# Daaohame/RAHT-3DGS-codec

Measured on AMD Instinct MI355X. Metric: M-Gaussians/s fwd+inv RAHT, 59-ch SH3 3DGS, higher is better.
Workload: dtype f32 (xyz columns: f64); 1 GPU; cfg3: 2999072 Gaussians (3000000 draws/GPU, J=12, 59 channels), fwd RAHT + quantize/reorder + dequantize/un-reorder + inv RAHT (quantization fused into the transform kernels); the 3 xyz columns carried in float64 inside the same launches (raht_fwd_quant_mixed / raht_dequant_inv_mixed): the reference's integers on every column; rows_per_gpu=2999072, channels=59, depth_J=12, engine=tile, quantize=True, parallelism=1 GPU, world=1

## Files before the change

raht-3dgs-codec_amd/csrc/transform_mx.hip:

```cpp
#include "raht_common.h"
#include "raht_device.h"
#include "tile_engine.h"
#include "tile_host.h"

#include <algorithm>
#include <cstdlib>
#include <string>
#include <type_traits>
#include <vector>

namespace raht {

#ifdef RAHT_PHASE_CLOCKS
constexpr int MX_CLK_TILES = 4096, MX_CLK_SLOTS = 12;
__device__ unsigned long long g_phase_clk_mx[MX_CLK_TILES][MX_CLK_SLOTS];
#define MX_STAMP(k) do { if (IDENT && threadIdx.x == 0 && tile_id < MX_CLK_TILES) g_phase_clk_mx[tile_id][k] = __builtin_readcyclecounter(); } while (0)
#else
#define MX_STAMP(k) do { } while (0)
#endif

constexpr int MX_MAX_WIDE = 4;
constexpr int MX_THREADS = 512;
constexpr int MX_TOP_THREADS = 1024;
constexpr int MX_TOP_SLOTS = RAHT_TOP_MAX_ROWS / MX_TOP_THREADS;

struct StepTableMX {
    StepTable f;
    double w[MX_MAX_WIDE];
};

static size_t tile_lds_bytes_mx(int R, int NF, int nwide)
{
    const size_t data = (size_t)R * NF * 16 + (((size_t)R * nwide * 8 + 15) & ~(size_t)15);
    const size_t meta = (size_t)R * (16 + 4 + 4);
    const size_t surv = ((size_t)R * 2 + 15) & ~(size_t)15;
    return data + meta + surv;
}

struct MxPtrs {
    const double *in_w;
    double *out_w;
    double *wsn_w;
    double *root_w;
    const uint32_t *prog;
    uint32_t prog_stride, prog_ab;
    int prog_compact;
};

struct MxMultiQ {
    int k;
    uint32_t fast_div;
    double step[MULTI_Q_MAX];
    int32_t *Q[MULTI_Q_MAX];
};

template <bool INV, bool IDENT, int SLOTS, bool ROOTS, bool MULTI = false, bool SQ = false>
__device__ __forceinline__ void tile_body_mx(const TileArgs<float> &A, const MxPtrs &P, const StepTableMX &ST, const int64_t tile_id,
                                             const MxMultiQ *MQ = nullptr)
{
    extern __shared__ __align__(16) unsigned char smem[];
    typedef RegChunk<float> V16;
    typedef RegChunk<double> W16;
    typedef RegChunk<int32_t> I16;
    const int R = A.R;
    const int tid0 = threadIdx.x;
    const int nthreads = blockDim.x, nwv = nthreads >> 6;
    const int nwide = A.nwide;
    const int lgw = nwide > 2 ? 2 : nwide - 1;
    const int Df = A.D;
    const int Fp = A.Dp, NF = Fp >> 2;
    const int lg = A.lg, lr = 6 - A.lg;
    const uint32_t NFm = ((1u << 20) + (uint32_t)NF - 1) / (uint32_t)NF;
    auto sync_lds = [&]() { asm volatile("s_waitcnt lgkmcnt(0)\n\ts_barrier" ::: "memory"); };
    auto wait_landed = [&]() { asm volatile("s_waitcnt vmcnt(0)" ::: "memory"); };

    size_t off = 0;
    float *ftile = (float *)smem; off += (size_t)R * Fp * 4;
    double *wd = (double *)(smem + off); off += ((size_t)R * nwide * 8 + 15) & ~(size_t)15;
    W16 *rec_ab = (W16 *)(smem + off); off += (size_t)R * 16;
    uint32_t *rec_pj = (uint32_t *)(smem + off); off += (size_t)R * 4;
    int32_t *sdst = (int32_t *)(smem + off); off += (size_t)R * 4;
    uint16_t *ssurv = (uint16_t *)(smem + off);

    auto lane_geom = [&](int tid, int &lane, int &wid, int &g, int &c4, int &fl, int &sp, int &goff, bool &head) {
        lane = tid & 63;
        wid = __builtin_amdgcn_readfirstlane(tid >> 6);
        g = lane >> lg;
        c4 = lane & ((1 << lg) - 1);
        fl = min(c4, NF - 1);
        head = c4 == 0;
        sp = fl;
        goff = min(fl * 4, Df - 4);
    };
    float my_step[4], my_rcp[4], tab_step[4];
    auto fetch_steps = [&](int place) {
        const int g0 = ST.f.n == 1 ? 0 : min(place * 4, Df - 4);
#pragma unroll
        for (int i = 0; i < 4; ++i) tab_step[i] = ST.f.v[g0 + i];
    };
    auto use_steps = [&]() {
#pragma unroll
        for (int i = 0; i < 4; ++i) {
            my_step[i] = ST.f.n == 1 ? ST.f.v[0] : tab_step[i];
            my_rcp[i] = refined_rcp(my_step[i]);
        }
    };

    int tid = tid0;
    asm volatile("" : "+v"(tid));
    int lane, wid, g, c4, fl, sp, goff; bool head;
    lane_geom(tid, lane, wid, g, c4, fl, sp, goff, head);
    const int64_t e0 = tile_id * R;
    const int nt = (int)min((int64_t)R, A.n_entries - e0);
    MX_STAMP(0);
    if constexpr (!MULTI) fetch_steps(fl);

    const uint32_t *pg = P.prog + (uint64_t)tile_id * P.prog_stride;
    const int end_v = ((const uint16_t *)pg)[lane];
    const int endm_v = lane ? ((const uint16_t *)pg)[lane - 1] : 0;
    uint32_t surv_raw = A.surv_off ? A.surv_off[tile_id + (tid0 & 1)] : 0u;
    uint32_t m_rw[SLOTS], m_rec[SLOTS];
    W16 m_ab[SLOTS];
#pragma unroll
    for (int s = 0; s < SLOTS; ++s) {
        const int j = tid0 + s * nthreads;
        m_rw[s] = 0; m_rec[s] = 0; m_ab[s].v[0] = 0.0; m_ab[s].v[1] = 0.0;
        if (j < nt) {
            m_rw[s] = pg[32 + j];
            m_rec[s] = pg[32 + R + j];
            if (!P.prog_compact) m_ab[s] = ((const W16 *)(pg + P.prog_ab))[j];
        }
    }
    auto early_loads_landed = [&]() {
        asm volatile("" : "+v"(surv_raw));
        if constexpr (!MULTI) asm volatile("" : "+v"(tab_step[0]), "+v"(tab_step[1]), "+v"(tab_step[2]), "+v"(tab_step[3]));
    };
    auto fin_of = [&](uint32_t rw) { return (rw >> 31) != 0 || (A.last_stage && !ROOTS); };
    auto write_dst = [&]() {
#pragma unroll
        for (int s = 0; s < SLOTS; ++s) {
            const int j = tid0 + s * nthreads;
            if (j < nt) sdst[j] = (int32_t)((m_rw[s] & 0x7fffffffu) | (fin_of(m_rw[s]) ? 0x80000000u : 0u));
        }
    };
    auto write_survivors = [&](uint32_t n_merged) {
#pragma unroll
        for (int s = 0; s < SLOTS; ++s) {
            const uint32_t k = (uint32_t)(tid0 + s * nthreads);
            if (k >= n_merged && k < (uint32_t)nt) ssurv[k - n_merged] = (uint16_t)m_rec[s];
        }
    };
    auto write_records = [&](uint32_t n_merged) {
#pragma unroll
        for (int s = 0; s < SLOTS; ++s) {
            const uint32_t k = (uint32_t)(tid0 + s * nthreads);
            if (k < n_merged) {
                uint32_t pj = m_rec[s];
                W16 ab = m_ab[s];
                if (P.prog_compact) {
                    const uint32_t j = pj & 1023u, l = (pj >> 10) & 1023u, r = (pj >> 20) & 1023u;
                    const double w0 = (double)(int)l, w1 = (double)(int)r;
                    const double den = w0 + w1;
                    ab.v[0] = sqrt(w0 / den);
                    ab.v[1] = sqrt(w1 / den);
                    pj = (j - l) | (j << 16);
                }
                rec_ab[k] = ab;
                rec_pj[k] = pj;
            }
        }
    };

    auto load_linear = [&](const float *dst, int chunks, const float *src) {
        const uint32_t lds0 = (uint32_t)(uintptr_t)(__attribute__((address_space(3))) const void *)dst;
        for (int it = wid; (it << 6) < chunks; it += nwv) {
            const int c = (it << 6) + lane;
            if (c < chunks) glds16<0>(src + (uint32_t)c * 4u, lds0 + ((uint32_t)it << 10));
        }
    };
    auto load_caller_rows = [&](int rows, auto src) {
        const uint32_t lds0 = (uint32_t)(uintptr_t)(__attribute__((address_space(3))) const void *)ftile;
        const int total = rows * NF;
        for (int it = wid; (it << 6) < total; it += nwv) {
            const int c = (it << 6) + lane;
            const int jr = (int)(((uint32_t)c * NFm) >> 20), ch = c - jr * NF;
            if (c < total) { const void *a = src(jr, (uint32_t)min(ch * 4, Df - 4)); if (a) glds16<1>(a, lds0 + ((uint32_t)it << 10)); }
        }
    };
    auto widen_row = [&](int j) {
        double *row = wd + __mul24(j, nwide);
        const V16 raw = *(const V16 *)(ftile + __mul24(j, Fp));
        double d[4];
#pragma unroll
        for (int i = 0; i < 4; ++i) d[i] = i < nwide ? (double)raw.v[i] : 0.0;
#pragma unroll
        for (int i = 0; i < 4; ++i) if (i < nwide) row[i] = d[i];
    };

    if constexpr (!INV) {
        if constexpr (IDENT) {
            const uint32_t ldc = (uint32_t)A.ld_in;
            const float *src = A.in + e0 * (int64_t)ldc;
            load_caller_rows(nt, [&](int jr, uint32_t go) { return row_at(src, (uint32_t)jr, ldc, go); });
        } else {
            load_linear(ftile, nt * NF, A.in + e0 * (int64_t)Fp);
            load_linear((const float *)wd, (nt * nwide + 1) >> 1, (const float *)(P.in_w + e0 * (int64_t)nwide));
        }
        MX_STAMP(9);
        const uint32_t n_merged = (uint32_t)__builtin_amdgcn_readlane(end_v, 63);
        write_dst();
        write_survivors(n_merged);
        write_records(n_merged);
        MX_STAMP(1);
        wait_landed();
        early_loads_landed();
        sync_lds();
        MX_STAMP(2);
        if constexpr (IDENT) {
#pragma unroll
            for (int s = 0; s < SLOTS; ++s) {
                const int j = tid + s * nthreads;
                if (j < nt) widen_row(j);
            }
            sync_lds();
        }
        MX_STAMP(3);
        MX_STAMP(4);
    } else {
        const uint32_t n_merged = (uint32_t)__builtin_amdgcn_readlane(end_v, 63);
        write_dst();
        write_survivors(n_merged);
        MX_STAMP(1);
        sync_lds();
        MX_STAMP(2);
        load_caller_rows(nt, [&](int jr, uint32_t go) -> const void * {
            const uint32_t d = (uint32_t)sdst[jr];
            return (d >> 31) ? (const void *)row_far((const int32_t *)A.Q, d & 0x7fffffffu, (uint32_t)A.ldq, go) : nullptr; });
        write_records(n_merged);
        const uint32_t surv_base = (uint32_t)__builtin_amdgcn_readlane((int)surv_raw, 0);
        const uint32_t surv_cnt = (uint32_t)__builtin_amdgcn_readlane((int)surv_raw, 1) - surv_base;
        if (!A.last_stage) {
            if (c4 < NF) for (uint32_t it = wid; (it << lr) < surv_cnt; it += nwv) {
                const uint32_t qc = min((it << lr) + g, surv_cnt - 1);
                const V16 x = ld_chunk<float>(row_at((const float *)A.wsn + (int64_t)surv_base * Fp, qc, (uint32_t)Fp, (uint32_t)(fl * 4)));
                *(V16 *)&ftile[__mul24((int)ssurv[qc], Fp) + fl * 4] = x;
            }
            for (uint32_t c = (uint32_t)tid; c < surv_cnt * (uint32_t)nwide; c += (uint32_t)nthreads) {
                const uint32_t qc = c / (uint32_t)nwide, i = c - qc * (uint32_t)nwide;
                wd[__mul24((int)ssurv[qc], nwide) + i] = P.wsn_w[(int64_t)surv_base * nwide + c];
            }
        } else if (ROOTS) {
            if (c4 < NF) for (uint32_t it = wid; (it << lr) < surv_cnt; it += nwv) {
                const uint32_t qc = min((it << lr) + g, surv_cnt - 1);
                const V16 x = ld_chunk<float>(A.root_buf + (int64_t)(surv_base + qc) * Df + goff);
                *(V16 *)&ftile[__mul24((int)ssurv[qc], Fp) + fl * 4] = x;
            }
            for (uint32_t c = (uint32_t)tid; c < surv_cnt * (uint32_t)nwide; c += (uint32_t)nthreads) {
                const uint32_t qc = c / (uint32_t)nwide, i = c - qc * (uint32_t)nwide;
                wd[__mul24((int)ssurv[qc], nwide) + i] = P.root_w[(int64_t)surv_base * nwide + c];
            }
        }
        MX_STAMP(3);
        wait_landed();
        early_loads_landed();
        sync_lds();
        MX_STAMP(4);
        use_steps();
#pragma unroll
        for (int s = 0; s < SLOTS; ++s) {
            const int j = tid0 + s * nthreads;
            if (j < nt && fin_of(m_rw[s])) {
                double *row = wd + __mul24(j, nwide);
                const I16 raw = *(const I16 *)(ftile + __mul24(j, Fp));
#pragma unroll
                for (int i = 0; i < 4; ++i) if (i < nwide) row[i] = (double)raw.v[i] * ST.w[i];
            }
        }
        if (A.last_stage && !ROOTS) {
            const uint32_t n_fin = (uint32_t)nt - n_merged;
            if (c4 < NF) for (uint32_t it = wid; (it << lr) < n_fin; it += nwv) {
                const uint32_t qc = (it << lr) + g;
                if (qc < n_fin) {
                    V16 *pr = (V16 *)&ftile[__mul24((int)ssurv[qc], Fp) + fl * 4];
                    const I16 raw = *(const I16 *)pr;
                    V16 x;
#pragma unroll
                    for (int i = 0; i < 4; ++i)
                        x.v[i] = (head && i < nwide) ? __int_as_float(raw.v[i]) : (float)raw.v[i] * my_step[i];
                    *pr = x;
                }
            }
        }
        sync_lds();
    }
    MX_STAMP(5);
    {
        const uint32_t stride = (uint32_t)(nwv << lr);
        const uint32_t gw = (uint32_t)lane >> lgw, cw = (uint32_t)min(lane & ((1 << lgw) - 1), nwide - 1);
        const uint32_t bw = 64u >> lgw;
        const uint32_t cf = (uint32_t)fl * 4u;
        bool chained = false;
        const int loff_v = endm_v, hist_v = end_v - endm_v;
        uint64_t mask = __ballot(hist_v > 0);
        while (mask) {
            const int l = INV ? (63 - __clzll((long long)mask)) : (__ffsll((long long)mask) - 1);
            mask &= ~(1ull << l);
            const uint32_t base = (uint32_t)__builtin_amdgcn_readlane(loff_v, l), cnt = (uint32_t)__builtin_amdgcn_readlane(hist_v, l);
            auto apply_f = [&](auto UC, uint32_t mb) {
                constexpr int U = decltype(UC)::value;
                W16 ab[U];
                uint32_t pj[U];
#pragma unroll
                for (int u = 0; u < U; ++u) { const uint32_t m = base + min(mb + u * stride + g, cnt - 1); pj[u] = rec_pj[m]; ab[u] = rec_ab[m]; }
                uint32_t ip[U], ij[U];
                V16 x0[U], x1[U];
#pragma unroll
                for (int u = 0; u < U; ++u) { ip[u] = __umul24(pj[u] & 0xffffu, (uint32_t)Fp) + cf; ij[u] = __umul24(pj[u] >> 16, (uint32_t)Fp) + cf; }
#pragma unroll
                for (int u = 0; u < U; ++u) { x0[u] = *(const V16 *)&ftile[ip[u]]; x1[u] = *(const V16 *)&ftile[ij[u]]; }
                if constexpr (INV) {
#pragma unroll
                    for (int u = 0; u < U; ++u) {
#pragma unroll
                        for (int i = 0; i < 4; ++i) x1[u].v[i] = (float)__float_as_int(x1[u].v[i]) * my_step[i];
                    }
                }
#pragma unroll
                for (int u = 0; u < U; ++u) {
                    const float ca = (float)ab[u].v[0], cb = (float)ab[u].v[1];
                    V16 lo, hi;
#pragma unroll
                    for (int i = 0; i < 4; ++i) {
                        if (!INV) {
                            lo.v[i] = ca * x0[u].v[i] + cb * x1[u].v[i];
                            hi.v[i] = ca * x1[u].v[i] - cb * x0[u].v[i];
                        } else {
                            lo.v[i] = ca * x0[u].v[i] - cb * x1[u].v[i];
                            hi.v[i] = cb * x0[u].v[i] + ca * x1[u].v[i];
                        }
                    }
                    if (u == 0 || mb + u * stride < cnt) { *(V16 *)&ftile[ip[u]] = lo; *(V16 *)&ftile[ij[u]] = hi; }
                }
            };
            auto pass_f = [&](auto UC) {
                constexpr int U = decltype(UC)::value;
                for (uint32_t mb = (uint32_t)(wid << lr); mb < cnt; mb += stride * U) apply_f(UC, mb);
            };
            auto apply_w = [&](uint32_t m0) {
                const uint32_t m = base + min(m0 + gw, cnt - 1);
                const uint32_t pj = rec_pj[m];
                const W16 ab = rec_ab[m];
                const uint32_t ip = __umul24(pj & 0xffffu, (uint32_t)nwide) + cw, ij = __umul24(pj >> 16, (uint32_t)nwide) + cw;
                const double d0 = wd[ip], d1 = wd[ij];
                const double ca = ab.v[0], cb = ab.v[1];
                double lo, hi;
                if (!INV) {
                    lo = ca * d0 + cb * d1;
                    hi = ca * d1 - cb * d0;
                } else {
                    lo = ca * d0 - cb * d1;
                    hi = cb * d0 + ca * d1;
                }
                wd[ip] = lo; wd[ij] = hi;
            };
            if (cnt <= (1u << lr)) {
                if (wid == 0) pass_f(std::integral_constant<int, 1>());
                else if (wid == 1) { for (uint32_t m0 = 0; m0 < cnt; m0 += bw) apply_w(m0); }
                chained = true;
            } else {
                if (chained) { __syncthreads(); chained = false; }
                if (cnt <= stride) pass_f(std::integral_constant<int, 1>());
                else pass_f(std::integral_constant<int, TILE_ROUND_U>());
                for (uint32_t m0 = (uint32_t)(nwv - 1 - wid) * bw; m0 < cnt; m0 += (uint32_t)nwv * bw) apply_w(m0);
                __syncthreads();
            }
        }
        if (chained) __syncthreads();
    }

    MX_STAMP(6);
    {
        int tid5 = tid0;
        asm volatile("" : "+v"(tid5));
        lane_geom(tid5, lane, wid, g, c4, fl, sp, goff, head);
    }
    const bool rowlane = c4 < NF;
    if constexpr (INV) {
        if constexpr (IDENT) {
            float *base = A.out + e0 * A.ld_out;
            double acc[4] = {0.0, 0.0, 0.0, 0.0};
            const float *rbase = SQ ? A.ref + e0 * A.ld_ref : nullptr;
            if (rowlane) for (int it = wid; (it << lr) < nt; it += 2 * nwv) {
                int j[2]; V16 x[2]; double w[2][4] = {};
                V16 c[2];
                if constexpr (SQ) {
#pragma unroll
                    for (int u = 0; u < 2; ++u)
                        c[u] = ld_chunk<float, true>(row_at(rbase, (uint32_t)min(((it + u * nwv) << lr) + g, nt - 1), (uint32_t)A.ld_ref, (uint32_t)goff));
                }
#pragma unroll
                for (int u = 0; u < 2; ++u) {
                    j[u] = min(((it + u * nwv) << lr) + g, nt - 1);
                    x[u] = *(const V16 *)&ftile[__mul24(j[u], Fp) + sp * 4];
                }
                if (head) {
#pragma unroll
                    for (int u = 0; u < 2; ++u) {
#pragma unroll
                        for (int i = 0; i < 4; ++i) w[u][i] = wd[__mul24(j[u], nwide) + min(i, nwide - 1)];
                    }
                }
                asm volatile("" : "+v"(w[0][0]), "+v"(w[0][1]), "+v"(w[0][2]), "+v"(w[0][3]), "+v"(w[1][0]), "+v"(w[1][1]), "+v"(w[1][2]), "+v"(w[1][3]));
#pragma unroll
                for (int u = 0; u < 2; ++u) {
#pragma unroll
                    for (int i = 0; i < 4; ++i) { const float f = (float)w[u][i]; x[u].v[i] = (head && i < nwide) ? f : x[u].v[i]; }
                    asm volatile("" : "+v"(x[u].v[0]), "+v"(x[u].v[1]), "+v"(x[u].v[2]), "+v"(x[u].v[3]));
                    if constexpr (SQ) {
                        if (u == 0 || ((it + nwv) << lr) < nt) {
                            if (A.out) st_chunk<float, true>(row_at(base, (uint32_t)j[u], (uint32_t)A.ld_out, (uint32_t)goff), x[u]);
                            if (((it + u * nwv) << lr) + g < nt) {
#pragma unroll
                                for (int i = 0; i < 4; ++i) { const float d = x[u].v[i] - c[u].v[i]; acc[i] += (double)d * (double)d; }
                            }
                        }
                    } else if (u == 0 || ((it + nwv) << lr) < nt) {
                        st_chunk<float, true>(row_at(base, (uint32_t)j[u], (uint32_t)A.ld_out, (uint32_t)goff), x[u]);
                    }
                }
            }
            if constexpr (SQ) {
#pragma unroll
                for (int i = 0; i < 4; ++i) {
                    for (int sh = 1 << lg; sh < 64; sh <<= 1) acc[i] += __shfl_xor(acc[i], sh, 64);
                }
                __syncthreads();
                double *sacc = (double *)smem;
                if (g == 0 && rowlane) {
#pragma unroll
                    for (int i = 0; i < 4; ++i) sacc[(wid * NF + c4) * 4 + i] = acc[i];
                }
                __syncthreads();
                if (tid0 < NF * 4) {
                    double t = 0.0;
                    for (int w = 0; w < nwv; ++w) t += sacc[w * NF * 4 + tid0];
                    A.sq_part[tile_id * (NF * 4) + tid0] = t;
                }
            }
        } else {
            float *bf = A.out + e0 * (int64_t)Fp;
            double *bw_ = P.out_w + e0 * (int64_t)nwide;
            for (int c = tid; c < nt * NF; c += nthreads) st_chunk<float>(bf + c * 4, *(const V16 *)&ftile[c * 4]);
            for (int c = tid; c < nt * nwide; c += nthreads) bw_[c] = wd[c];
        }
    } else {
        if (!A.last_stage || ROOTS) {
            const uint32_t surv_base = (uint32_t)__builtin_amdgcn_readlane((int)surv_raw, 0);
            const uint32_t surv_cnt = (uint32_t)__builtin_amdgcn_readlane((int)surv_raw, 1) - surv_base;
            constexpr bool to_roots = ROOTS;
            float *bf = to_roots ? A.root_buf + (int64_t)surv_base * Df : A.wsn + (int64_t)surv_base * Fp;
            double *bw_ = (to_roots ? P.root_w : P.wsn_w) + (int64_t)surv_base * nwide;
            const uint32_t ldb = (uint32_t)(to_roots ? Df : Fp), cb = (uint32_t)(to_roots ? goff : fl * 4);
            if (c4 < NF) for (uint32_t it = wid; (it << lr) < surv_cnt; it += nwv) {
                const uint32_t q = min((it << lr) + g, surv_cnt - 1);
                const V16 x = *(const V16 *)&ftile[__mul24((int)ssurv[q], Fp) + fl * 4];
                st_chunk<float>(row_at(bf, q, ldb, cb), x);
            }
            for (uint32_t c = (uint32_t)tid; c < surv_cnt * (uint32_t)nwide; c += (uint32_t)nthreads) {
                const uint32_t q = c / (uint32_t)nwide, i = c - q * (uint32_t)nwide;
                bw_[c] = wd[__mul24((int)ssurv[q], nwide) + i];
            }
        }
        if constexpr (MULTI) {
            int32_t *qa = (int32_t *)rec_ab;
            auto store_step = [&](auto fast_div, int32_t *Qd) {
                if (rowlane) for (int it = wid; (it << lr) < nt; it += 2 * nwv) {
                    int jc[2]; V16 x[2]; I16 qi[2] = {}; uint32_t dv[2];
#pragma unroll
                    for (int u = 0; u < 2; ++u) {
                        jc[u] = min(((it + u * nwv) << lr) + g, nt - 1);
                        x[u] = *(const V16 *)&ftile[__mul24(jc[u], Fp) + sp * 4];
                        dv[u] = (uint32_t)sdst[jc[u]];
                    }
                    if (head) {
#pragma unroll
                        for (int u = 0; u < 2; ++u) {
#pragma unroll
                            for (int i = 0; i < 4; ++i) qi[u].v[i] = qa[__mul24(jc[u], nwide) + min(i, nwide - 1)];
                        }
                    }
                    asm volatile("" : "+v"(x[0].v[0]), "+v"(x[1].v[0]), "+v"(qi[0].v[0]), "+v"(qi[0].v[1]), "+v"(qi[0].v[2]), "+v"(qi[0].v[3]),
                                 "+v"(qi[1].v[0]), "+v"(qi[1].v[1]), "+v"(qi[1].v[2]), "+v"(qi[1].v[3]));
#pragma unroll
                    for (int u = 0; u < 2; ++u) {
                        I16 qv;
#pragma unroll
                        for (int i = 0; i < 4; ++i) {
                            const int32_t q = quantize_one(x[u].v[i], my_step[i], my_rcp[i], decltype(fast_div)::value);
                            qv.v[i] = (head && i < nwide) ? qi[u].v[i] : q;
                        }
                        asm volatile("" : "+v"(qv.v[0]), "+v"(qv.v[1]), "+v"(qv.v[2]), "+v"(qv.v[3]));
                        if ((dv[u] >> 31) && (u == 0 || ((it + nwv) << lr) < nt))
                            st_chunk<int32_t, true>(row_far(Qd, dv[u] & 0x7fffffffu, (uint32_t)A.ldq, (uint32_t)goff), qv);
                    }
                }
            };
            for (int kk = 0; kk < MQ->k; ++kk) {
                const double sw = MQ->step[kk];
#pragma unroll
                for (int s = 0; s < SLOTS; ++s) {
                    const int j = tid0 + s * nthreads;
                    if (j < nt && ((uint32_t)sdst[j] >> 31)) {
                        const double *row = &wd[__mul24(j, nwide)];
                        int32_t *qrow = &qa[__mul24(j, nwide)];
#pragma unroll
                        for (int i = 0; i < 4; ++i) if (i < nwide) qrow[i] = quantize_one_f64(row[i], sw);
                    }
                }
                sync_lds();
                const float sf = (float)sw, rf = refined_rcp(sf);
#pragma unroll
                for (int i = 0; i < 4; ++i) { my_step[i] = sf; my_rcp[i] = rf; }
                if ((MQ->fast_div >> kk) & 1u) store_step(std::true_type(), MQ->Q[kk]);
                else store_step(std::false_type(), MQ->Q[kk]);
                sync_lds();
            }
        } else {
            MX_STAMP(10);
#pragma unroll
            for (int s = 0; s < SLOTS; ++s) {
                const int j = tid0 + s * nthreads;
                if (j < nt && ((uint32_t)sdst[j] >> 31)) {
                    double *row = &wd[__mul24(j, nwide)];
                    double d[4] = {0.0, 0.0, 0.0, 0.0};
#pragma unroll
                    for (int i = 0; i < 4; ++i) if (i < nwide) d[i] = row[i];
                    asm volatile("" ::: "memory");
                    int32_t *qrow = (int32_t *)row;
#pragma unroll
                    for (int i = 0; i < 4; ++i) if (i < nwide) qrow[i] = quantize_one_f64(d[i], ST.w[i]);
                }
            }
            sync_lds();
            MX_STAMP(7);
            use_steps();
#ifdef RAHT_PHASE_CLOCKS
            asm volatile("" :: "v"(my_step[0]), "v"(my_rcp[3]));
#endif
            MX_STAMP(11);
            auto store_final = [&](auto fast_div) {
                if (rowlane) for (int it = wid; (it << lr) < nt; it += 2 * nwv) {
                    int jc[2]; V16 x[2]; I16 qi[2] = {}; uint32_t dv[2];
#pragma unroll
                    for (int u = 0; u < 2; ++u) {
                        jc[u] = min(((it + u * nwv) << lr) + g, nt - 1);
                        x[u] = *(const V16 *)&ftile[__mul24(jc[u], Fp) + sp * 4];
                        dv[u] = (uint32_t)sdst[jc[u]];
                    }
                    if (head) {
#pragma unroll
                        for (int u = 0; u < 2; ++u) {
                            const int32_t *qrow = (const int32_t *)&wd[__mul24(jc[u], nwide)];
#pragma unroll
                            for (int i = 0; i < 4; ++i) qi[u].v[i] = qrow[min(i, nwide - 1)];
                        }
                    }
                    asm volatile("" : "+v"(x[0].v[0]), "+v"(x[1].v[0]), "+v"(qi[0].v[0]), "+v"(qi[0].v[1]), "+v"(qi[0].v[2]), "+v"(qi[0].v[3]),
                                 "+v"(qi[1].v[0]), "+v"(qi[1].v[1]), "+v"(qi[1].v[2]), "+v"(qi[1].v[3]));
#pragma unroll
                    for (int u = 0; u < 2; ++u) {
                        I16 qv;
#pragma unroll
                        for (int i = 0; i < 4; ++i) {
                            const int32_t q = quantize_one(x[u].v[i], my_step[i], my_rcp[i], decltype(fast_div)::value);
                            qv.v[i] = (head && i < nwide) ? qi[u].v[i] : q;
                        }
                        asm volatile("" : "+v"(qv.v[0]), "+v"(qv.v[1]), "+v"(qv.v[2]), "+v"(qv.v[3]));
                        if ((dv[u] >> 31) && (u == 0 || ((it + nwv) << lr) < nt))
                            st_chunk<int32_t, true>(row_far(A.Q, dv[u] & 0x7fffffffu, (uint32_t)A.ldq, (uint32_t)goff), qv);
                    }
                }
            };
            if (ST.f.fast_div) store_final(std::true_type()); else store_final(std::false_type());
        }
    }
    MX_STAMP(8);
}

template <bool INV, bool IDENT, int SLOTS>
__global__ __launch_bounds__(MX_THREADS, 6) void tile_kernel_mx(const TileArgs<float> A, const MxPtrs P, const StepTableMX ST)
{
    tile_body_mx<INV, IDENT, SLOTS, false>(A, P, ST, (int64_t)blockIdx.x);
}
template <bool INV, bool IDENT, int SLOTS>
__global__ __launch_bounds__(MX_THREADS, 6) void tile_kernel_mx_roots(const TileArgs<float> A, const MxPtrs P, const StepTableMX ST)
{
    tile_body_mx<INV, IDENT, SLOTS, true>(A, P, ST, (int64_t)blockIdx.x);
}
template <bool IDENT, int SLOTS>
__global__ __launch_bounds__(MX_THREADS, 6) void tile_kernel_mx_multi(const TileArgs<float> A, const MxPtrs P, const StepTableMX ST, const MxMultiQ M)
{
    tile_body_mx<false, IDENT, SLOTS, false, true, false>(A, P, ST, (int64_t)blockIdx.x, &M);
}
template <int SLOTS>
__global__ __launch_bounds__(MX_THREADS, 6) void tile_kernel_mx_sq(const TileArgs<float> A, const MxPtrs P, const StepTableMX ST)
{
    tile_body_mx<true, true, SLOTS, false, false, true>(A, P, ST, (int64_t)blockIdx.x);
}

struct TileBatchMX {
    TileArgs<float> a[BATCH_MAX];
    MxPtrs p[BATCH_MAX];
    uint32_t first_tile[BATCH_MAX + 1];
    int n;
};
static_assert(sizeof(TileBatchMX) + sizeof(StepTableMX) <= 4096, "tile_kernel_mx_batch: arguments exceed the 4 KB kernarg segment");

template <bool INV, bool IDENT, int SLOTS>
__global__ __launch_bounds__(MX_THREADS, 6) void tile_kernel_mx_batch(const TileBatchMX B, const StepTableMX ST)
{
    int s = 0;
#pragma unroll
    for (int q = 1; q < BATCH_MAX; ++q) s += (q < B.n && blockIdx.x >= B.first_tile[q]) ? 1 : 0;
    tile_body_mx<INV, IDENT, SLOTS, false>(B.a[s], B.p[s], ST, (int64_t)(blockIdx.x - B.first_tile[s]));
}

struct TopArgsMX {
    const float *in_rows;  int64_t ld_in;
    const float *in_img; const double *in_img_w;
    float *out_rows;       int64_t ld_out;
    float *out_img; double *out_img_w;
    int32_t *Q;            int64_t ldq;
    const uint32_t *e_pos;
    const uint32_t *pj;
    const float *ab32;  const double *ab64;
    int n, n_merges, D, nwide, Fp;
    const uint32_t *lev;
    int nlev, nbig;
    uint32_t small_start;
    const uint32_t *root_rank;
    float *root_f; double *root_w;
};

template <bool WIDE, bool INV, bool ROOTS, bool MULTI = false>
__device__ __forceinline__ void top_body_mx(const TopArgsMX &A, const StepTableMX &ST, const int chunk, const MxMultiQ *MQ = nullptr)
{
    typedef typename std::conditional<WIDE, double, float>::type T;
    constexpr int VN = WIDE ? 2 : 4;
    typedef RegChunk<T> V16;
    extern __shared__ __align__(16) unsigned char smem[];
    V16 *tile = (V16 *)smem;
    __shared__ uint32_t s_lev[2 * 64];
    const int tid = threadIdx.x;
    const int nwide = A.nwide;
    const int goff = WIDE ? 2 * chunk : min(chunk * 4, A.D - 4);
    const int ioff = chunk * 4;
    const int n = A.n, nm = A.n_merges;
    if (tid < 2 * A.nlev) s_lev[tid] = A.lev[tid];
    const T *ab = WIDE ? (const T *)A.ab64 : (const T *)A.ab32;
    const int n_small = nm - (int)A.small_start;
    uint32_t *s_pj = (uint32_t *)(smem + (size_t)n * 16);
    T *s_ab = (T *)(s_pj + ((n_small + 3) & ~3));
    for (int i = tid; i < n_small; i += MX_TOP_THREADS) {
        s_pj[i] = A.pj[A.small_start + i];
        s_ab[2 * i] = ab[2 * (A.small_start + i)];
        s_ab[2 * i + 1] = ab[2 * (A.small_start + i) + 1];
    }
    T my_step[VN];
    float my_rcp[VN];
    bool live[VN];
#pragma unroll
    for (int i = 0; i < VN; ++i) {
        if constexpr (WIDE) { live[i] = goff + i < nwide; my_step[i] = live[i] ? ST.w[goff + i] : 1.0; my_rcp[i] = 1.0f; }
        else { live[i] = !(chunk == 0 && i < nwide); my_step[i] = ST.f.v[ST.f.n == 1 ? 0 : goff + i]; my_rcp[i] = refined_rcp(my_step[i]); }
    }
    uint32_t pj[MX_TOP_SLOTS];
    T ra[MX_TOP_SLOTS], rb[MX_TOP_SLOTS];
#pragma unroll
    for (int k = 0; k < MX_TOP_SLOTS; ++k) {
        const int idx = min(k * MX_TOP_THREADS + tid, max(nm - 1, 0));
        pj[k] = A.pj[idx]; ra[k] = ab[2 * idx]; rb[k] = ab[2 * idx + 1];
    }
    uint32_t m_dst[MX_TOP_SLOTS], m_rr[MX_TOP_SLOTS];
#pragma unroll
    for (int k = 0; k < MX_TOP_SLOTS; ++k) {
        m_dst[k] = A.e_pos[min(k * MX_TOP_THREADS + tid, n - 1)];
        m_rr[k] = ROOTS ? A.root_rank[min(k * MX_TOP_THREADS + tid, n - 1)] : 0xffffffffu;
    }
#pragma unroll
    for (int k = 0; k < MX_TOP_SLOTS; ++k) {
        const int e = k * MX_TOP_THREADS + tid;
        if (e >= n) continue;
        V16 v;
        if constexpr (!INV) {
            if (A.in_img) {
                if constexpr (WIDE) {
#pragma unroll
                    for (int i = 0; i < VN; ++i) v.v[i] = live[i] ? A.in_img_w[(int64_t)e * nwide + goff + i] : 0.0;
                } else {
                    v = *(const V16 *)(A.in_img + (int64_t)e * A.Fp + ioff);
                }
            } else if constexpr (WIDE) {
#pragma unroll
                for (int i = 0; i < VN; ++i) v.v[i] = live[i] ? (double)A.in_rows[(int64_t)e * A.ld_in + goff + i] : 0.0;
            } else {
                v = ld_chunk<float>(A.in_rows + (int64_t)e * A.ld_in + goff);
            }
        } else if (m_rr[k] != 0xffffffffu) {
            if constexpr (WIDE) {
#pragma unroll
                for (int i = 0; i < VN; ++i) v.v[i] = live[i] ? A.root_w[(int64_t)m_rr[k] * nwide + goff + i] : 0.0;
            } else {
                v = ld_chunk<float>(A.root_f + (int64_t)m_rr[k] * A.D + goff);
            }
        } else {
            const int32_t *q = A.Q + (int64_t)m_dst[k] * A.ldq + goff;
            if constexpr (WIDE) {
#pragma unroll
                for (int i = 0; i < VN; ++i) v.v[i] = live[i] ? (double)q[i] * my_step[i] : 0.0;
            } else {
                const RegChunk<int32_t> raw = ld_chunk<int32_t>(q);
#pragma unroll
                for (int i = 0; i < VN; ++i) v.v[i] = (float)raw.v[i] * my_step[i];
            }
        }
        tile[e] = v;
    }
    __syncthreads();

    auto butterfly = [&](uint32_t rec, T a, T b) {
        const uint32_t ip = rec & 0xffffu, ij = rec >> 16;
        const V16 x0 = tile[ip], x1 = tile[ij];
        V16 vlo, vhi;
#pragma unroll
        for (int i = 0; i < VN; ++i) {
            if (!INV) {
// ... 608 lines not shown
}

template <bool INV>
static int run_batch_mx(const char *what, int n, raht_plan *const *plans, const MxIO *ios, int D, const double *steps, int n_steps,
                        int n_wide, hipStream_t s)
{
    std::vector<MxScene> scn((size_t)n);
    for (int i = 0; i < n; ++i) {
        const MxIO &io = ios[i];
        const void *a = INV ? (const void *)io.Q : (const void *)io.C_in, *b = INV ? (const void *)io.C_out : (const void *)io.Q;
        RAHT_RET(mx_batch_check_plan(what, i, plans[i], a, b, D, INV ? io.ldq : io.ldc, INV ? io.ldc : io.ldq, steps, n_steps, n_wide));
    }
    std::vector<size_t> first((size_t)n + 1, 0);
    for (int i = 0; i < n; ++i) {
        MxScene &S = scn[(size_t)i];
        S.p = plans[i]; S.io = ios[i];
        Schedule *sc = nullptr;
        RAHT_RET(mx_setup(S.p, D, n_wide, std::max(S.io.ldc, S.io.ldq), s, &sc, S.g));
        S.sc = mx_batchable(S.p, sc) ? sc : nullptr;
        first[(size_t)i + 1] = first[(size_t)i] + (S.sc ? S.sc->stages.size() : 0);
    }
    std::vector<MxStageLaunch> prep(first[(size_t)n]);
    for (int i = 0; i < n; ++i) {
        const MxScene &S = scn[(size_t)i];
        if (!S.sc) continue;
        for (int k = 0; k < (int)S.sc->stages.size(); ++k) {
            const int rc = prepare_stage_mx<INV>(S.p, *S.sc, k, S.io, D, S.g, prep[first[(size_t)i] + (size_t)k]);
            if (rc != RAHT_OK) {
                const std::string msg = raht_last_error();
                set_error("%s: %s (scene %d)", what, msg.c_str(), i);
                return rc;
            }
        }
    }
    StepTableMX stp;
    fill_steps_mx(stp, steps, n_steps, n_wide);
    auto stage_of = [&](int i, int k) -> const MxStageLaunch & { return prep[first[(size_t)i] + (size_t)k]; };
    auto single = [&](int i) -> int {
        const MxIO &io = scn[(size_t)i].io;
        if constexpr (INV) return dequant_inv_mixed_impl(scn[(size_t)i].p, io.Q, io.ldq, D, steps, n_steps, n_wide, io.C_out, io.ldc, (raht_stream_t)s);
        else return fwd_quant_mixed_impl(scn[(size_t)i].p, io.C_in, io.ldc, D, steps, n_steps, n_wide, io.Q, io.ldq, (raht_stream_t)s);
    };
    auto tile = [&](int m, const int *idx, int k) -> int {
        if (m == 1) return launch_prepared_mx<INV>(scn[(size_t)idx[0]].p, k, scn[(size_t)idx[0]].io, stage_of(idx[0], k), scn[(size_t)idx[0]].g, stp, s);
        const MxStageLaunch *Ls[BATCH_MAX];
        for (int q = 0; q < m; ++q) Ls[q] = &stage_of(idx[q], k);
        return launch_tile_batch_mx<INV>(m, Ls, k == 0, stp, s);
    };
    auto top = [&](int m, const int *idx, int k) -> int {
        if (m == 1) return launch_prepared_mx<INV>(scn[(size_t)idx[0]].p, k, scn[(size_t)idx[0]].io, stage_of(idx[0], k), scn[(size_t)idx[0]].g, stp, s);
        const MxStageLaunch *Ls[BATCH_MAX];
        for (int q = 0; q < m; ++q) Ls[q] = &stage_of(idx[q], k);
        return launch_top_batch_mx<INV>(m, Ls, scn[(size_t)idx[0]].g.NCp, stp, s);
    };
    BatchCounts cnt;
    return group_mx_scenes<INV>(n, scn.data(), cnt, single, tile, top);
}

static int mixed_batch_stats_impl(int n, raht_plan *const *plans, int D, int n_wide, int inverse, int *tile_launches, int *top_launches,
                                  int *single_scene_calls)
{
    const char *what = "raht_mixed_batch_stats";
    if (n < 1 || !plans || !tile_launches || !top_launches || !single_scene_calls || D < 1 || n_wide < 1 || n_wide > MX_MAX_WIDE || n_wide > D) {
        set_error("%s: bad argument", what);
        return RAHT_ERR_INVALID;
    }
    RAHT_RET(check_batch_plans(what, n, plans));
    std::vector<MxScene> scn((size_t)n);
    for (int i = 0; i < n; ++i) {
        MxScene &S = scn[(size_t)i];
        S.p = plans[i];
        RAHT_RET(check_plan_device(S.p, what));
        if (S.p->row_map) { set_error("%s: not available for row-mapped plans (scene %d)", what, i); return RAHT_ERR_UNSUPPORTED; }
        Schedule *sc = nullptr;
        RAHT_RET(mx_setup(S.p, D, n_wide, D, nullptr, &sc, S.g));
        S.sc = mx_batchable(S.p, sc) ? sc : nullptr;
    }
    BatchCounts cnt;
    auto none1 = [](int) { return (int)RAHT_OK; };
    auto none3 = [](int, const int *, int) { return (int)RAHT_OK; };
    if (inverse) RAHT_RET((group_mx_scenes<true>(n, scn.data(), cnt, none1, none3, none3)));
    else RAHT_RET((group_mx_scenes<false>(n, scn.data(), cnt, none1, none3, none3)));
    *tile_launches = cnt.tile; *top_launches = cnt.top; *single_scene_calls = cnt.single;
    return RAHT_OK;
}

}

using namespace raht;

extern "C" {

int raht_fwd_quant_mixed(const raht_plan *plan, const float *C, int64_t ldc, int D, const double *steps, int n_steps, int n_wide,
                         int32_t *Q, int64_t ldq, raht_stream_t stream)
{
    return guarded("raht_fwd_quant_mixed", [&]() { return fwd_quant_mixed_impl(plan, C, ldc, D, steps, n_steps, n_wide, Q, ldq, stream); });
}

int raht_dequant_inv_mixed(const raht_plan *plan, const int32_t *Q, int64_t ldq, int D, const double *steps, int n_steps, int n_wide,
                           float *C, int64_t ldc, raht_stream_t stream)
{
    return guarded("raht_dequant_inv_mixed", [&]() { return dequant_inv_mixed_impl(plan, Q, ldq, D, steps, n_steps, n_wide, C, ldc, stream); });
}

int raht_fwd_quant_mixed_multi(const raht_plan *plan, const float *C, int64_t ldc, int D, const double *steps, int k, int n_wide,
                               int32_t *const *Q, int64_t ldq, raht_stream_t stream)
{
    return guarded("raht_fwd_quant_mixed_multi", [&]() { return fwd_quant_mixed_multi_impl(plan, C, ldc, D, steps, k, n_wide, Q, ldq, stream); });
}

int raht_dequant_inv_mixed_sqdiff(const raht_plan *plan, const int32_t *Q, int64_t ldq, int D, const double *steps, int n_steps,
                                  int n_wide, const float *C_ref, int64_t ld_ref, float *C_rec, int64_t ldc, double *sqdiff,
                                  raht_stream_t stream)
{
    return guarded("raht_dequant_inv_mixed_sqdiff", [&]() {
        return dequant_inv_mixed_sqdiff_impl(plan, Q, ldq, D, steps, n_steps, n_wide, C_ref, ld_ref, C_rec, ldc, sqdiff, stream); });
}

int raht_fwd_quant_mixed_batch(int n, raht_plan *const *plans, const float *const *C, const int64_t *ldc, int D,
                               const double *steps, int n_steps, int n_wide, int32_t *const *Q, const int64_t *ldq, raht_stream_t stream)
{
    const char *what = "raht_fwd_quant_mixed_batch";
    return guarded(what, [&]() -> int {
        RAHT_RET(mx_batch_check_args(what, n, plans, (const void *const *)C, ldc, (const void *const *)Q, ldq, D, steps, n_steps, n_wide));
        std::vector<MxIO> ios((size_t)n);
        for (int i = 0; i < n; ++i) { MxIO &io = ios[(size_t)i]; io.C_in = C[i]; io.ldc = ldc[i]; io.Q = Q[i]; io.ldq = ldq[i]; }
        return run_batch_mx<false>(what, n, plans, ios.data(), D, steps, n_steps, n_wide, (hipStream_t)stream);
    });
}

int raht_dequant_inv_mixed_batch(int n, raht_plan *const *plans, const int32_t *const *Q, const int64_t *ldq, int D,
                                 const double *steps, int n_steps, int n_wide, float *const *C, const int64_t *ldc, raht_stream_t stream)
{
    const char *what = "raht_dequant_inv_mixed_batch";
    return guarded(what, [&]() -> int {
        RAHT_RET(mx_batch_check_args(what, n, plans, (const void *const *)Q, ldq, (const void *const *)C, ldc, D, steps, n_steps, n_wide));
        std::vector<MxIO> ios((size_t)n);
        for (int i = 0; i < n; ++i) { MxIO &io = ios[(size_t)i]; io.C_out = C[i]; io.ldc = ldc[i]; io.Q = const_cast<int32_t *>(Q[i]); io.ldq = ldq[i]; }
        return run_batch_mx<true>(what, n, plans, ios.data(), D, steps, n_steps, n_wide, (hipStream_t)stream);
    });
}

int raht_mixed_batch_stats(int n, raht_plan *const *plans, int D, int n_wide, int inverse, int *tile_launches, int *top_launches,
                           int *single_scene_calls)
{
    return guarded("raht_mixed_batch_stats", [&]() {
        return mixed_batch_stats_impl(n, plans, D, n_wide, inverse, tile_launches, top_launches, single_scene_calls); });
}

#ifdef RAHT_PHASE_CLOCKS
int raht_debug_read_phase_clocks_mx(unsigned long long *dst, int n_tiles)
{
    RAHT_HIP_CHECK(hipDeviceSynchronize());
    RAHT_HIP_CHECK(hipMemcpyFromSymbol(dst, HIP_SYMBOL(g_phase_clk_mx), sizeof(unsigned long long) * MX_CLK_SLOTS * (size_t)std::min(n_tiles, MX_CLK_TILES)));
    return MX_CLK_SLOTS;
}
#endif

int raht_plan_mixed_stats(raht_plan *plan, int D, int n_wide, int *tile_rows, int *n_stages, int64_t *rows_per_stage, int max_stages)
{
    return guarded("raht_plan_mixed_stats", [&]() -> int {
        if (!plan || !tile_rows || !n_stages || D < 1 || n_wide < 1 || n_wide > MX_MAX_WIDE) { set_error("raht_plan_mixed_stats: bad argument"); return RAHT_ERR_INVALID; }
        RAHT_RET(check_plan_device(plan, "raht_plan_mixed_stats"));
        *tile_rows = 0; *n_stages = 0;
        if (plan->row_map) return RAHT_OK;
        Schedule *sc = nullptr;
        MxGeom g;
        RAHT_RET(mx_setup(plan, D, n_wide, D, nullptr, &sc, g));
        if (!sc) return RAHT_OK;
        *tile_rows = g.R0;
        *n_stages = (int)sc->stages.size();
        for (int k = 0; k < *n_stages && k < max_stages && rows_per_stage; ++k) rows_per_stage[k] = sc->stages[(size_t)k].n_entries;
        return RAHT_OK;
    });
}

}
```

Baseline: 4917 M-Gaussians/s.

## Overlap forward final quantize/store with trailing chained merge rounds

In the forward non-multi path, quantization and store of merged rows now begin for rows finalized before the last wide merge round. While waves 0-1 run the trailing single-wave chained merges, the remaining waves write those rows, and the trailing barrier after the chain is dropped. The separate f64 quantize pass and its LDS sync are folded into a per-block write_rows routine that walks rows in merge-record order, followed by survivors and late rows. Phase-clock instrumentation is also extended. The rewrite depends on record-order indexing being correct and brings more complex control flow and register use.

```diff
diff --git a/raht-3dgs-codec_amd/csrc/transform_mx.hip b/raht-3dgs-codec_amd/csrc/transform_mx.hip
--- a/raht-3dgs-codec_amd/csrc/transform_mx.hip
+++ b/raht-3dgs-codec_amd/csrc/transform_mx.hip
@@ -12,10 +12,12 @@
 namespace raht {
 
 #ifdef RAHT_PHASE_CLOCKS
-constexpr int MX_CLK_TILES = 4096, MX_CLK_SLOTS = 12;
-__device__ unsigned long long g_phase_clk_mx[MX_CLK_TILES][MX_CLK_SLOTS];
-#define MX_STAMP(k) do { if (IDENT && threadIdx.x == 0 && tile_id < MX_CLK_TILES) g_phase_clk_mx[tile_id][k] = __builtin_readcyclecounter(); } while (0)
+constexpr int MX_CLK_TILES = 4096, MX_CLK_LATER = 1024, MX_CLK_SLOTS = 16;
+__device__ unsigned long long g_phase_clk_mx[MX_CLK_TILES + MX_CLK_LATER][MX_CLK_SLOTS];
+#define MX_STAMP_SET(k, val) do { if (threadIdx.x == 0 && tile_id < (IDENT ? MX_CLK_TILES : MX_CLK_LATER)) g_phase_clk_mx[(IDENT ? 0 : MX_CLK_TILES) + tile_id][k] = (val); } while (0)
+#define MX_STAMP(k) MX_STAMP_SET(k, __builtin_readcyclecounter())
 #else
+#define MX_STAMP_SET(k, val) do { } while (0)
 #define MX_STAMP(k) do { } while (0)
 #endif
 
@@ -294,6 +296,9 @@
         sync_lds();
     }
     MX_STAMP(5);
+#ifdef RAHT_PHASE_CLOCKS
+    uint32_t clk_rounds = 0, clk_chain = 0;
+#endif
     {
         const uint32_t stride = (uint32_t)(nwv << lr);
         const uint32_t gw = (uint32_t)lane >> lgw, cw = (uint32_t)min(lane & ((1 << lgw) - 1), nwide - 1);
@@ -364,10 +369,18 @@
                 wd[ip] = lo; wd[ij] = hi;
             };
             if (cnt <= (1u << lr)) {
+#ifdef RAHT_PHASE_CLOCKS
+                if (!INV && !chained) MX_STAMP(12);
+                ++clk_chain;
+#endif
                 if (wid == 0) pass_f(std::integral_constant<int, 1>());
                 else if (wid == 1) { for (uint32_t m0 = 0; m0 < cnt; m0 += bw) apply_w(m0); }
                 chained = true;
             } else {
+#ifdef RAHT_PHASE_CLOCKS
+                if (INV && chained) MX_STAMP(12);
+                ++clk_rounds;
+#endif
                 if (chained) { __syncthreads(); chained = false; }
                 if (cnt <= stride) pass_f(std::integral_constant<int, 1>());
                 else pass_f(std::integral_constant<int, TILE_ROUND_U>());
@@ -375,10 +388,11 @@
                 __syncthreads();
             }
         }
-        if (chained) __syncthreads();
+        if constexpr (INV || MULTI) { if (chained) __syncthreads(); }
     }
 
     MX_STAMP(6);
+    MX_STAMP_SET(15, (unsigned long long)clk_rounds | ((unsigned long long)clk_chain << 8));
     {
         int tid5 = tid0;
         asm volatile("" : "+v"(tid5));
@@ -454,7 +468,60 @@
             for (int c = tid; c < nt * nwide; c += nthreads) bw_[c] = wd[c];
         }
     } else {
-        if (!A.last_stage || ROOTS) {
+        const uint32_t n_merged5 = (uint32_t)__builtin_amdgcn_readlane(end_v, 63);
+        auto write_rows = [&](auto fast_div, const uint32_t w, const uint32_t nw, const uint32_t lo, const uint32_t hi) __attribute__((always_inline)) {
+            auto slot_of = [&](uint32_t q) { return q < n_merged5 ? rec_pj[q] >> 16 : (uint32_t)ssurv[q - n_merged5]; };
+            const uint32_t blk = max(16u, 1u << lr);
+            const uint32_t ga = (uint32_t)lane >> 2, ca = (uint32_t)min(lane & 3, nwide - 1);
+            double ws[4] = {ST.w[0], ST.w[1], ST.w[2], ST.w[3]};
+            asm volatile("" : "+s"(ws[0]), "+s"(ws[1]), "+s"(ws[2]), "+s"(ws[3]));
+            const double wstep = ca == 0 ? ws[0] : ca == 1 ? ws[1] : ca == 2 ? ws[2] : ws[3];
+            for (uint32_t b0 = lo + w * blk; b0 < hi; b0 += nw * blk) {
+                const uint32_t be = min(b0 + blk, hi);
+                for (uint32_t q0 = b0; q0 < be; q0 += 16u) {
+                    if (q0 + ga < be) {
+                        int32_t *qrow = (int32_t *)&wd[__umul24(slot_of(q0 + ga), (uint32_t)nwide)];
+                        const double d = ((const double *)qrow)[ca];
+                        asm volatile("" ::: "memory");
+                        qrow[ca] = quantize_one_f64(d, wstep);
+                    }
+                }
+                asm volatile("" ::: "memory");
+                if (rowlane) for (uint32_t r0 = b0; r0 < be; r0 += 2u << lr) {
+                    int jc[2]; V16 x[2]; I16 qi[2] = {}; uint32_t dv[2];
+#pragma unroll
+                    for (int u = 0; u < 2; ++u) {
+                        jc[u] = (int)slot_of(min(r0 + ((uint32_t)u << lr) + (uint32_t)g, be - 1));
+                        x[u] = *(const V16 *)&ftile[__mul24(jc[u], Fp) + sp * 4];
+                        dv[u] = (uint32_t)sdst[jc[u]];
+                    }
+                    if (head) {
+#pragma unroll
+                        for (int u = 0; u < 2; ++u) {
+                            const int32_t *qrow = (const int32_t *)&wd[__mul24(jc[u], nwide)];
+#pragma unroll
+                            for (int i = 0; i < 4; ++i) qi[u].v[i] = qrow[min(i, nwide - 1)];
+                        }
+                    }
+                    asm volatile("" : "+v"(x[0].v[0]), "+v"(x[1].v[0]), "+v"(qi[0].v[0]), "+v"(qi[0].v[1]), "+v"(qi[0].v[2]), "+v"(qi[0].v[3]),
+                                 "+v"(qi[1].v[0]), "+v"(qi[1].v[1]), "+v"(qi[1].v[2]), "+v"(qi[1].v[3]));
+#pragma unroll
+                    for (int u = 0; u < 2; ++u) {
+                        I16 qv;
+#pragma unroll
+                        for (int i = 0; i < 4; ++i) {
+                            const int32_t q = quantize_one(x[u].v[i], my_step[i], my_rcp[i], decltype(fast_div)::value);
+                            qv.v[i] = (head && i < nwide) ? qi[u].v[i] : q;
+                        }
+                        asm volatile("" : "+v"(qv.v[0]), "+v"(qv.v[1]), "+v"(qv.v[2]), "+v"(qv.v[3]));
+                        if (u == 0 || r0 + (1u << lr) < be)
+                            st_chunk<int32_t, true>(row_far(A.Q, dv[u] & 0x7fffffffu, (uint32_t)A.ldq, (uint32_t)goff), qv);
+                    }
+                }
+            }
+        };
+        auto store_survivors = [&]() __attribute__((always_inline)) {
+            if (A.last_stage && !ROOTS) return;
             const uint32_t surv_base = (uint32_t)__builtin_amdgcn_readlane((int)surv_raw, 0);
             const uint32_t surv_cnt = (uint32_t)__builtin_amdgcn_readlane((int)surv_raw, 1) - surv_base;
             constexpr bool to_roots = ROOTS;
@@ -470,8 +537,9 @@
                 const uint32_t q = c / (uint32_t)nwide, i = c - q * (uint32_t)nwide;
                 bw_[c] = wd[__mul24((int)ssurv[q], nwide) + i];
             }
-        }
+        };
         if constexpr (MULTI) {
+            store_survivors();
             int32_t *qa = (int32_t *)rec_ab;
             auto store_step = [&](auto fast_div, int32_t *Qd) {
                 if (rowlane) for (int it = wid; (it << lr) < nt; it += 2 * nwv) {
@@ -526,62 +594,27 @@
                 sync_lds();
             }
         } else {
-            MX_STAMP(10);
-#pragma unroll
-            for (int s = 0; s < SLOTS; ++s) {
-                const int j = tid0 + s * nthreads;
-                if (j < nt && ((uint32_t)sdst[j] >> 31)) {
-                    double *row = &wd[__mul24(j, nwide)];
-                    double d[4] = {0.0, 0.0, 0.0, 0.0};
-#pragma unroll
-                    for (int i = 0; i < 4; ++i) if (i < nwide) d[i] = row[i];
-                    asm volatile("" ::: "memory");
-                    int32_t *qrow = (int32_t *)row;
-#pragma unroll
-                    for (int i = 0; i < 4; ++i) if (i < nwide) qrow[i] = quantize_one_f64(d[i], ST.w[i]);
-                }
-            }
-            sync_lds();
-            MX_STAMP(7);
+            uint32_t k_late = 0;
+            const uint64_t wide_rounds = __ballot(end_v - endm_v > (1 << lr));
+            if (wide_rounds) k_late = (uint32_t)__builtin_amdgcn_readlane(end_v, 63 - __clzll((long long)wide_rounds));
+            const bool tail_chain = k_late < n_merged5;
+            const uint32_t n_late = n_merged5 + ((A.last_stage && !ROOTS) ? (uint32_t)nt - n_merged5 : 0u);
+            MX_STAMP_SET(15, (unsigned long long)clk_rounds | ((unsigned long long)clk_chain << 8) | ((unsigned long long)(n_merged5 - k_late) << 16));
             use_steps();
-#ifdef RAHT_PHASE_CLOCKS
-            asm volatile("" :: "v"(my_step[0]), "v"(my_rcp[3]));
-#endif
-            MX_STAMP(11);
-            auto store_final = [&](auto fast_div) {
-                if (rowlane) for (int it = wid; (it << lr) < nt; it += 2 * nwv) {
-                    int jc[2]; V16 x[2]; I16 qi[2] = {}; uint32_t dv[2];
-#pragma unroll
-                    for (int u = 0; u < 2; ++u) {
-                        jc[u] = min(((it + u * nwv) << lr) + g, nt - 1);
-                        x[u] = *(const V16 *)&ftile[__mul24(jc[u], Fp) + sp * 4];
-                        dv[u] = (uint32_t)sdst[jc[u]];
+            auto finish = [&](auto fast_div) __attribute__((always_inline)) {
+#pragma nounroll
+                for (int late = 0; late < 2; ++late) {
+                    if (late) {
+                        if (tail_chain) __syncthreads();
+                        MX_STAMP(13);
+                        store_survivors();
+                        MX_STAMP(7);
                     }
-                    if (head) {
-#pragma unroll
-                        for (int u = 0; u < 2; ++u) {
-                            const int32_t *qrow = (const int32_t *)&wd[__mul24(jc[u], nwide)];
-#pragma unroll
-                            for (int i = 0; i < 4; ++i) qi[u].v[i] = qrow[min(i, nwide - 1)];
-                        }
-                    }
-                    asm volatile("" : "+v"(x[0].v[0]), "+v"(x[1].v[0]), "+v"(qi[0].v[0]), "+v"(qi[0].v[1]), "+v"(qi[0].v[2]), "+v"(qi[0].v[3]),
-                                 "+v"(qi[1].v[0]), "+v"(qi[1].v[1]), "+v"(qi[1].v[2]), "+v"(qi[1].v[3]));
-#pragma unroll
-                    for (int u = 0; u < 2; ++u) {
-                        I16 qv;
-#pragma unroll
-                        for (int i = 0; i < 4; ++i) {
-                            const int32_t q = quantize_one(x[u].v[i], my_step[i], my_rcp[i], decltype(fast_div)::value);
-                            qv.v[i] = (head && i < nwide) ? qi[u].v[i] : q;
-                        }
-                        asm volatile("" : "+v"(qv.v[0]), "+v"(qv.v[1]), "+v"(qv.v[2]), "+v"(qv.v[3]));
-                        if ((dv[u] >> 31) && (u == 0 || ((it + nwv) << lr) < nt))
-                            st_chunk<int32_t, true>(row_far(A.Q, dv[u] & 0x7fffffffu, (uint32_t)A.ldq, (uint32_t)goff), qv);
-                    }
+                    const uint32_t w0 = (!late && tail_chain) ? 2u : 0u;
+                    if ((uint32_t)wid >= w0) write_rows(fast_div, (uint32_t)wid - w0, (uint32_t)nwv - w0, late ? k_late : 0u, late ? n_late : k_late);
                 }
             };
-            if (ST.f.fast_div) store_final(std::true_type()); else store_final(std::false_type());
+            if (ST.f.fast_div) finish(std::true_type()); else finish(std::false_type());
         }
     }
     MX_STAMP(8);
@@ -1496,7 +1529,7 @@
 int raht_debug_read_phase_clocks_mx(unsigned long long *dst, int n_tiles)
 {
     RAHT_HIP_CHECK(hipDeviceSynchronize());
-    RAHT_HIP_CHECK(hipMemcpyFromSymbol(dst, HIP_SYMBOL(g_phase_clk_mx), sizeof(unsigned long long) * MX_CLK_SLOTS * (size_t)std::min(n_tiles, MX_CLK_TILES)));
+    RAHT_HIP_CHECK(hipMemcpyFromSymbol(dst, HIP_SYMBOL(g_phase_clk_mx), sizeof(unsigned long long) * MX_CLK_SLOTS * (size_t)std::min(n_tiles, MX_CLK_TILES + MX_CLK_LATER)));
     return MX_CLK_SLOTS;
 }
 #endif
```

After: 4372 M-Gaussians/s. 11.1% lower.
